# mikostrzewa/AprilSLAM

Hardware: AMD Instinct MI355X
Metric: frames/sec at 1280x720, 20 tags/frame (detection + batched PnP) (higher is better)
Workload: dtype u8/f64

## Files before the change

aprilslam_amd/csrc/aprilslam.hip:

```cpp
#include "../../include/aprilslam.h"

#include <algorithm>
#include <chrono>
#include <cmath>
#include <cstdarg>
#include <cstdio>
#include <cstring>
#include <memory>
#include <string>
#include <type_traits>
#include <vector>

#include "asl_common.h"
#include "tag_standard41h12.inc"
#include "k_wave.inc"

#include "k_threshold.inc"
#include "k_blur.inc"
#include "k_cc.inc"
#include "k_cluster.inc"
#include "k_seg.inc"
#include "k_quad.inc"
#include "k_decode.inc"
#include "k_pnp.inc"
// ... 70 lines not shown
    DevBuf<uint8_t> bgray;
    const uint8_t *qgray = nullptr;
    DevBuf<uint8_t> dbg_thresh;
    DevBuf<unsigned int> dbg_labels;
    DevBuf<unsigned int> parent, sizes;
    DevBuf<unsigned long long> hkeys, points, rootmask, wmask, bmask;
    DevBuf<unsigned int> hcounts, class_lists, stage_pos, frame_cursor, dense_tiles, dense_seg, quad_list;
    DevBuf<unsigned long long> stage_rec;
    DevBuf<uint4> seg_edges;
    unsigned int stage_cap = 0;
    DevBuf<unsigned long long> slot_cluster;
    DevBuf<ClusterRec> clusters;
    DevBuf<QuadRec> quads;
    DevBuf<double> scratch, quadH, wtab, side_mom;
    DevBuf<DetRec> dets;
    DevBuf<unsigned int> frame_ndets, frame_idx, frame_nkeep, frame_off;
    DevBuf<DetOut> out_det;
    DevBuf<PoseOut> out_pose;
    DevBuf<long long> counters;
    DevBuf<float> pnp_corners;
    DevBuf<double> pnp_out;
    DevBuf<uint8_t> pnp_ok;
    DevBuf<uint8_t> gn_ws;
    DevBuf<uint8_t> loc_obs, loc_map;
    DevBuf<uint8_t> solve_out;
    DevBuf<uint8_t> rig_cams;
    DevBuf<uint8_t> cal_ws;
    DevBuf<uint8_t> map_ws, map_lm;
    hipStream_t copy_stream = nullptr, host_stream = nullptr;
    std::vector<hipEvent_t> copy_done;
    hipStream_t aux_stream = nullptr;

    Geom last{};
    unsigned int nslots = 0, max_clusters = 0, max_points = 0, max_dets = 0;
    long long last_counters[CNT__N] = {0};
    bool pending = false;
    const uint8_t *p_frames = nullptr;
    Geom p_geom{};
    hipStream_t p_stream = nullptr;
    bool p_has_cam = false;
    CamDev p_cam{};
    size_t prefetched = 0, nd_guess = 0;
    std::chrono::steady_clock::time_point t_submit, t_enqueued;
    PinnedBuf<long long> pinned_counters;
    PinnedBuf<DetOut> host_det;
    PinnedBuf<PoseOut> host_pose;
    PinnedBuf<unsigned int> host_nkeep;

    int profiling = 0;
    hipEvent_t ev[MAX_STAGES + 1] = {nullptr};
    int nev = 0;
    const char *stage_names[MAX_STAGES] = {nullptr};
    float stage_ms[MAX_STAGES] = {0};
    int nstages = 0;
    float host_ms[4] = {0, 0, 0, 0};

    size_t host_cap() const { return std::min(host_det.n, host_pose.n); }
    ~asl_detector()
    {
        for (hipStream_t s : {aux_stream, copy_stream, host_stream})
            if (s) (void)hipStreamDestroy(s);
        for (hipEvent_t e : copy_done) (void)hipEventDestroy(e);
        for (hipEvent_t e : ev)
            if (e) (void)hipEventDestroy(e);
    }
};

static const char *kVersion = "aprilslam 0.1 gfx950 (HIP, tagStandard41h12)";

extern "C" const char *asl_last_error(void) { return g_err.c_str(); }
extern "C" const char *asl_version(void) { return kVersion; }

// ... 56 lines not shown
    d->fam.nbits = kTag41h12NBits;
    d->fam.width_at_border = kTag41h12WidthAtBorder;
    d->fam.total_width = kTag41h12TotalWidth;
    d->fam.reversed_border = 1;
    d->fam.ncodes = kTag41h12PinnedIds;
    for (int i = 0; i < kTag41h12NBits; i++) { d->fam.bit_x[i] = kTag41h12BitX[i]; d->fam.bit_y[i] = kTag41h12BitY[i]; }
    if (d->codes.ensure(kTag41h12NCodes)) return fail(ASL_ENOMEM, "hipMalloc(code book) failed");
    if (hipMemcpy(d->codes.p, kTag41h12Codes, sizeof(unsigned long long) * kTag41h12NCodes, hipMemcpyHostToDevice) != hipSuccess)
        return fail(ASL_EDEVICE, "hipMemcpy(code book) failed");
    d->fam.codes = d->codes.p;
    if (build_code_index(d.get())) return fail(ASL_ENOMEM, "code-book index allocation failed");
    if (d->wtab.ensure(WEIGHT_TABLE_N)) return fail(ASL_ENOMEM, "hipMalloc(weight table) failed");
    hipLaunchKernelGGL(k_weight_table, dim3((WEIGHT_TABLE_N + 255) / 256), dim3(256), 0, 0, d->wtab.p);
    if (hipDeviceSynchronize() != hipSuccess) return fail(ASL_EDEVICE, "weight table kernel failed");
    (void)hipFuncSetAttribute(reinterpret_cast<const void *>(&k_fit_quads<256, CLASS3_CAP / 256>), hipFuncAttributeMaxDynamicSharedMemorySize, QUAD_LDS_BYTES(CLASS3_CAP));
    *out = d.release();
    return ASL_OK;
}

extern "C" void asl_detector_destroy(asl_detector *d)
{
    if (!d) return;
    (void)hipSetDevice(d->device);
    if (d->pending) (void)hipStreamSynchronize(d->p_stream);
    delete d;
}

extern "C" int asl_detector_set_id_limit(asl_detector *d, int n_ids)
{
    if (!d) return fail(ASL_EINVAL, "detector is NULL");
// ... 53 lines not shown
}

extern "C" int asl_detector_set_pnp_both_minima(asl_detector *d, int enabled)
{
    if (!d) return fail(ASL_EINVAL, "detector is NULL");
    d->pnp_both_minima = enabled ? 1 : 0;
    return ASL_OK;
}

extern "C" int asl_set_profiling(asl_detector *d, int enabled)
{
    if (!d) return fail(ASL_EINVAL, "detector is NULL");
    d->profiling = enabled ? 1 : 0;
    if (enabled)
        for (int i = 0; i <= MAX_STAGES; i++)
            if (!d->ev[i]) HIPCHK(hipEventCreate(&d->ev[i]));
    return ASL_OK;
}

extern "C" int asl_stage_times(asl_detector *d, const char **names, float *ms, int max_n, int *n)
{
    if (!d || !n) return fail(ASL_EINVAL, "NULL argument");
    int k = std::min(max_n, d->nstages);
    for (int i = 0; i < k; i++) { if (names) names[i] = d->stage_names[i]; if (ms) ms[i] = d->stage_ms[i]; }
    static const char *hn[4] = {"host_enqueue", "host_wait", "host_copy", "host_post"};
    for (int i = 0; i < 4 && k < max_n; i++, k++) { if (names) names[k] = hn[i]; if (ms) ms[k] = d->host_ms[i]; }
    *n = k;
    return ASL_OK;
}

static int pnp_tpw(size_t expected)
// ... 61 lines not shown
    bad |= d->quads.ensure(d->max_clusters);
    bad |= d->quad_list.ensure(d->max_clusters);
    bad |= d->quadH.ensure((size_t)10 * d->max_clusters);
    bad |= d->side_mom.ensure((size_t)24 * d->max_clusters);
    bad |= d->points.ensure(d->max_points);
    d->stage_cap = (unsigned int)((double)g.npix * d->points_per_pixel) + 1024u;
    bad |= d->stage_rec.ensure((size_t)B * d->stage_cap);
    bad |= d->stage_pos.ensure((size_t)B * d->stage_cap);
    bad |= d->frame_cursor.ensure(B);
    bad |= d->dense_tiles.ensure(B * count_tiles(g));
    bad |= d->dense_seg.ensure(B * (size_t)seg_nwx(g) * (size_t)((g.sh + SEG_TH - 1) / SEG_TH));
    bad |= d->seg_edges.ensure(B * (size_t)seg_nwx(g) * (size_t)((g.sh + SEG_TH - 1) / SEG_TH));
    bad |= d->scratch.ensure((size_t)d->max_points * 8);
    bad |= d->dets.ensure(d->max_dets);
    bad |= d->frame_ndets.ensure(B);
    bad |= d->frame_nkeep.ensure(B);
    bad |= d->frame_off.ensure(B);
    bad |= d->frame_idx.ensure(B * (size_t)d->dets_per_frame);
    bad |= d->out_det.ensure(d->max_dets);
    bad |= d->out_pose.ensure(d->max_dets);
    bad |= d->counters.ensure(CNT__N);
    if (bad) return fail(ASL_ENOMEM, "device workspace allocation failed (%zu frames of %dx%d)", B, g.sw, g.sh);
    return ASL_OK;
}

#define STAGE(name)                                                        \
    do {                                                                   \
        if (d->profiling && d->nev < MAX_STAGES) {                         \
            d->stage_names[d->nev] = name;                                 \
            HIPCHK(hipEventRecord(d->ev[d->nev], st));                     \
            d->nev++;                                                      \
        }                                                                  \
    } while (0)

static int tag_width(const asl_detector *d, const Geom &g) { return std::max(3, d->fam.width_at_border / g.f); }

// ... 5 lines not shown
                       d->class_lists.p + (size_t)cls * d->max_clusters, d->counters.p, cls, d->max_clusters, CAP, d->points.p, d->qgray, g,
                       tag_width(d, g), want_rev, want_norm, d->scratch.p, d->quads.p, d->wtab.p, d->side_mom.p);
}

static void launch_fit_class(asl_detector *d, const Geom &g, int cls, unsigned int B, hipStream_t st)
{
    const unsigned int qgrid = std::min<unsigned int>(d->max_clusters, std::max<unsigned int>(16384u, 32u * B));
    const unsigned int q2grid = std::min<unsigned int>(d->max_clusters, 2048u);
    switch (cls) {
    case 0: return launch_fit<64, CLASS0_CAP>(d, g, 0, qgrid, st);
    case 1: return launch_fit<128, CLASS1_CAP>(d, g, 1, qgrid, st);
    case 2: return launch_fit<256, CLASS2_CAP>(d, g, 2, q2grid, st);
    case 3: return launch_fit<256, CLASS3_CAP>(d, g, 3, q2grid, st);
    default: return launch_fit<256, 0>(d, g, 4, q2grid, st);
    }
}

static void launch_quad_finish(asl_detector *d, const Geom &g, hipStream_t st)
{
    hipLaunchKernelGGL(k_quad_finish, dim3(std::min<unsigned int>((d->max_clusters + 63) / 64, 4096u)), dim3(256), 0, st, d->quads.p, d->side_mom.p, d->counters.p,
                       d->max_clusters, tag_width(d, g));
}

static int enqueue_detect(asl_detector *d, const uint8_t *d_frames, const Geom &g, hipStream_t st, const CamDev *cam)
{
    dim3 blk(64, 4, 1);
    int thx = (g.sh + TILESZ - 1) / TILESZ;
    unsigned int B = (unsigned int)g.nframes;
    d->nev = 0;
    range_push("S0-S4 gray, decimate, threshold, segmentation, clusters");
// ... 55 lines not shown
    hipLaunchKernelGGL((k_seg_points<SEGP_PCAP_DENSE, SEGP_RUNCAP_DENSE, 1, 2>), dim3(256), dim3(64), 0, st, d->wmask.p, d->bmask.p, g, nwx,
                       d->parent.p, d->sizes.p, d->hkeys.p, d->hcounts.p, d->nslots - 1, d->stage_rec.p, d->stage_pos.p, d->frame_cursor.p,
                       d->stage_cap, d->dense_tiles.p, pty, d->counters.p);
    STAGE("k_cluster_filter");
    hipLaunchKernelGGL(k_cluster_filter, dim3((d->nslots + 1023) / 1024), dim3(1024), 0, st, d->hkeys.p, d->hcounts.p, d->nslots, g,
                       d->clusters.p, d->slot_cluster.p, d->class_lists.p, d->max_clusters, d->max_points, d->counters.p);
    STAGE("k_point_place");
    hipLaunchKernelGGL(k_point_place, dim3(16, B), dim3(256), 0, st, d->stage_rec.p, d->stage_pos.p, d->frame_cursor.p, d->stage_cap,
                       d->slot_cluster.p, d->points.p, d->counters.p);

    range_pop();
    range_push("S5 quad fit");
    for (int cls = 0; cls < NCLASSES; cls++) {
        static const char *const kFitStage[NCLASSES] = {"k_fit_quads<0>", "k_fit_quads<1>", "k_fit_quads<2>", "k_fit_quads<3>", "k_fit_quads<4>"};
        STAGE(kFitStage[cls]);
        launch_fit_class(d, g, cls, B, st);
    }

    STAGE("k_quad_finish");
    launch_quad_finish(d, g, st);
    range_pop();
    range_push("S6-S7 edge refinement, homography, decode");
    STAGE("k_quad_compact");
    hipLaunchKernelGGL(k_quad_compact, dim3((d->max_clusters + 1023) / 1024), dim3(1024), 0, st, d->quads.p, d->counters.p, d->max_clusters,
                       d->quad_list.p);
    unsigned int dgrid = std::min<unsigned int>(d->max_clusters, std::max<unsigned int>(8192u, 64u * B));
    STAGE("k_refine");
    hipLaunchKernelGGL((g.channels == 1 ? k_refine<1> : k_refine<3>), dim3(dgrid), dim3(64), 0, st, d->quads.p, d->counters.p, d->max_clusters, d_frames, g,
                       d->fam.reversed_border ? 1 : 0, d->refine, d->quadH.p, d->quad_list.p, d->side_mom.p);
    STAGE("k_homography");
    hipLaunchKernelGGL(k_homography, dim3(std::min<unsigned int>((d->max_clusters + 31) / 32, 2048u)), dim3(256), 0, st, d->quadH.p, d->counters.p, d->max_clusters,
// ... 4 lines not shown

    range_pop();
    range_push("S9 PnP, S8 de-duplication");
    if (cam) {
        STAGE("k_pnp_dets");
        const int tpw = pnp_tpw(d->nd_guess ? d->nd_guess : (size_t)20 * B);
        hipLaunchKernelGGL(k_pnp_dets, dim3((d->max_dets + tpw - 1) / tpw), dim3(64), 0, st, d->dets.p, d->counters.p, d->max_dets, *cam, tpw);
    }
    STAGE("k_det_dedup");
    {
        const unsigned int cap_f = d->dets_per_frame;
        hipLaunchKernelGGL(k_det_bucket, dim3((d->max_dets + 255) / 256), dim3(256), 0, st, d->dets.p, d->counters.p, d->max_dets, d->frame_ndets.p,
                           d->frame_idx.p, cap_f, d->counters.p);
        hipLaunchKernelGGL(k_det_dedup, dim3(B), dim3(256), 0, st, d->dets.p, d->counters.p, d->frame_ndets.p, d->frame_idx.p, cap_f,
                           d->frame_nkeep.p, d->counters.p);
        hipLaunchKernelGGL(k_det_offsets, dim3(1), dim3(1024), 0, st, d->frame_nkeep.p, B, d->frame_off.p, d->counters.p);
        hipLaunchKernelGGL(k_det_gather, dim3((cap_f + 255) / 256, B), dim3(256), 0, st, d->dets.p, d->frame_idx.p, cap_f, d->frame_nkeep.p,
                           d->frame_off.p, d->out_det.p, d->out_pose.p, d->max_dets, cam ? 1 : 0);
    }
    range_pop();
    if (d->profiling && d->nev <= MAX_STAGES) HIPCHK(hipEventRecord(d->ev[d->nev], st));
    HIPCHK(hipGetLastError());
    return ASL_OK;
}

static CamDev make_cam(const asl_detector *d, const double *K, const double *dist, int n_dist, double tag_size)
{
    CamDev c;
    c.both_minima = d->pnp_both_minima; c.pad = 0;
    c.fx = K[0]; c.fy = K[4]; c.cx = K[2]; c.cy = K[5];
    c.k1 = c.k2 = c.p1 = c.p2 = c.k3 = 0;
    if (dist && n_dist >= 4) { c.k1 = dist[0]; c.k2 = dist[1]; c.p1 = dist[2]; c.p2 = dist[3]; }
    if (dist && n_dist >= 5) c.k3 = dist[4];
    c.half = (double)(float)(tag_size / 2);
    return c;
}

using clk = std::chrono::steady_clock;
static float msf(clk::time_point a, clk::time_point b) { return std::chrono::duration<float, std::milli>(b - a).count(); }

static int ensure_host_out(asl_detector *d, size_t want, size_t nframes)
{
    HIPCHK(d->host_nkeep.ensure(nframes, hipHostMallocDefault));
    if (want <= d->host_cap()) return ASL_OK;
    d->host_det.release(); d->host_pose.release();
    want = std::max<size_t>(want * 2, 4096);
    HIPCHK(d->host_det.ensure(want, hipHostMallocNonCoherent));
    HIPCHK(d->host_pose.ensure(want, hipHostMallocNonCoherent));
    return ASL_OK;
}

static int submit_batch(asl_detector *d, const uint8_t *d_frames, const Geom &g, hipStream_t st, const CamDev *cam)
{
    if (d->pending) return fail(ASL_EINVAL, "a batch is already in flight on this detector: collect it first");
    int rc = ensure_workspace(d, g);
    if (rc) return rc;
    d->t_submit = clk::now();
    rc = enqueue_detect(d, d_frames, g, st, cam);
    if (rc) return rc;
    HIPCHK(d->pinned_counters.ensure(CNT__N, hipHostMallocDefault));
    HIPCHK(hipMemcpyAsync(d->pinned_counters.p, d->counters.p, sizeof(long long) * CNT__N, hipMemcpyDeviceToHost, st));
    d->prefetched = 0;
    rc = ensure_host_out(d, std::min<size_t>(d->nd_guess, d->max_dets), (size_t)g.nframes);
    if (rc) return rc;
    HIPCHK(hipMemcpyAsync(d->host_nkeep.p, d->frame_nkeep.p, sizeof(unsigned int) * (size_t)g.nframes, hipMemcpyDeviceToHost, st));
    if (d->nd_guess > 0) {
        size_t guess = std::min<size_t>(d->nd_guess, d->max_dets);
        HIPCHK(hipMemcpyAsync(d->host_det.p, d->out_det.p, guess * sizeof(DetOut), hipMemcpyDeviceToHost, st));
        if (cam) HIPCHK(hipMemcpyAsync(d->host_pose.p, d->out_pose.p, guess * sizeof(PoseOut), hipMemcpyDeviceToHost, st));
        d->prefetched = guess;
    }
    d->pending = true;
    d->p_frames = d_frames; d->p_geom = g; d->p_stream = st; d->p_has_cam = cam != nullptr;
    if (cam) d->p_cam = *cam;
    d->t_enqueued = clk::now();
    return ASL_OK;
}

static int collect_batch(asl_detector *d, asl_detection *out, asl_pose *poses, int max_out, int *n_per_frame, int *n_out)
{
    if (!d->pending) return fail(ASL_EINVAL, "no batch in flight on this detector");
    const Geom g = d->p_geom;
    hipStream_t st = d->p_stream;
    const CamDev *cam = d->p_has_cam ? &d->p_cam : nullptr;
    clk::time_point t0 = d->t_submit, t1 = d->t_enqueued, t2 = t1;
    for (int attempt = 0; attempt < 4; attempt++) {
        if (attempt > 0) {
            d->pending = false;
            d->nd_guess = 0;
            int rc = submit_batch(d, d->p_frames, g, st, cam);
            if (rc) return rc;
        }
        HIPCHK(hipStreamSynchronize(st));
        t2 = clk::now();
        memcpy(d->last_counters, d->pinned_counters.p, sizeof(long long) * CNT__N);
        d->last = g;
        long long *c = d->last_counters;
        if (c[CNT_UF_GUARD]) {
            d->pending = false;
            return fail(ASL_ECAPACITY, "a union-find loop hit its iteration guard (%lld times): labels of this batch are not trustworthy", c[CNT_UF_GUARD]);
        }
        bool again = false;
        if (c[CNT_OVERFLOW_HASH]) { d->hash_slots_per_frame *= 4; again = true; }
        if (c[CNT_OVERFLOW_CLUSTERS] || c[CNT_NCLUSTERS] > (long long)d->max_clusters) { d->clusters_per_frame *= 4; again = true; }
        if (c[CNT_OVERFLOW_POINTS]) { d->points_per_pixel *= 2; again = true; }
        if (c[CNT_OVERFLOW_DETS]) { d->dets_per_frame *= 4; again = true; }
        if (again) {
            if (attempt == 3) {
                d->pending = false;
                return fail(ASL_ECAPACITY, "work buffers still overflow after growing (hash %lld clusters %lld points %lld dets %lld)",
// ... 1 lines not shown
            }
            continue;
        }
        break;
    }
    d->pending = false;
    if (d->profiling) {
        d->nstages = d->nev;
        for (int i = 0; i < d->nev; i++) HIPCHK(hipEventElapsedTime(&d->stage_ms[i], d->ev[i], d->ev[i + 1]));
    }
    if (d->last_counters[CNT_DEDUP_LIMIT])
        return fail(ASL_ECAPACITY, "%lld frame(s) hold more than %d detections: the de-duplication does not sort that many", d->last_counters[CNT_DEDUP_LIMIT], DEDUP_MAX);
    size_t nd = (size_t)d->last_counters[CNT_NKEEP];
    if (nd > d->max_dets) nd = d->max_dets;
    if (nd > d->prefetched) {
        size_t have = d->prefetched;
        if (nd > d->host_cap()) have = 0;
        int rc = ensure_host_out(d, nd, (size_t)g.nframes);
        if (rc) return rc;
        HIPCHK(hipMemcpy(d->host_det.p + have, d->out_det.p + have, (nd - have) * sizeof(DetOut), hipMemcpyDeviceToHost));
        if (cam) HIPCHK(hipMemcpy(d->host_pose.p + have, d->out_pose.p + have, (nd - have) * sizeof(PoseOut), hipMemcpyDeviceToHost));
    }
    d->nd_guess = nd + nd / 4 + 256;
    clk::time_point t3 = clk::now();
    static_assert(sizeof(DetOut) == sizeof(asl_detection) && sizeof(PoseOut) == sizeof(asl_pose), "device results are copied verbatim");
    int total = (int)nd;
    int nw = std::min(total, max_out);
    if (out && nw > 0) memcpy(out, d->host_det.p, (size_t)nw * sizeof(asl_detection));
    if (poses && cam && nw > 0) memcpy(poses, d->host_pose.p, (size_t)nw * sizeof(asl_pose));
    if (n_per_frame) for (int f = 0; f < g.nframes; f++) n_per_frame[f] = (int)d->host_nkeep.p[f];
    if (n_out) *n_out = total;
    d->host_ms[0] = msf(t0, t1); d->host_ms[1] = msf(t1, t2); d->host_ms[2] = msf(t2, t3); d->host_ms[3] = msf(t3, clk::now());
    return ASL_OK;
}

static int check_n_dist(int n_dist)
{
    if (n_dist != 0 && n_dist != 4 && n_dist != 5) return fail(ASL_EINVAL, "n_dist must be 0, 4 or 5");
    return ASL_OK;
}

static int check_device_args(asl_detector *d, const void *d_frames, int n_frames, int channels, int w, int h, int stride, size_t frame_pitch,
                             int n_dist, Geom *g)
{
    if (!d || !d_frames) return fail(ASL_EINVAL, "NULL detector or frames");
// ... 19 lines not shown
extern "C" int asl_collect_batch(asl_detector *d, asl_detection *out, asl_pose *poses, int max_out, int *n_per_frame, int *n_out)
{
    if (!d) return fail(ASL_EINVAL, "NULL detector");
    if (max_out < 0 || (max_out > 0 && !out)) return fail(ASL_EINVAL, "out is NULL");
    HIPCHK(hipSetDevice(d->device));
    return collect_batch(d, out, poses, max_out, n_per_frame, n_out);
}

extern "C" int asl_collect_batch_view(asl_detector *d, const asl_detection **out, const asl_pose **poses, const uint32_t **n_per_frame, int *n_out)
{
    if (!d || !out || !n_per_frame || !n_out) return fail(ASL_EINVAL, "NULL argument");
    HIPCHK(hipSetDevice(d->device));
    const bool with_poses = d->p_has_cam;
    int rc = collect_batch(d, nullptr, nullptr, 0, nullptr, n_out);
    if (rc) return rc;
    *out = reinterpret_cast<const asl_detection *>(d->host_det.p);
    if (poses) *poses = with_poses ? reinterpret_cast<const asl_pose *>(d->host_pose.p) : nullptr;
    *n_per_frame = d->host_nkeep.p;
    return ASL_OK;
}

extern "C" int asl_detect_batch_device(asl_detector *d, const void *d_frames, int n_frames, int channels, int w, int h, int stride,
                                       size_t frame_pitch, void *stream, const double *K, const double *dist, int n_dist,
                                       double tag_size, asl_detection *out, asl_pose *poses, int max_out, int *n_per_frame, int *n_out)
{
    if (max_out < 0 || (max_out > 0 && !out)) return fail(ASL_EINVAL, "out is NULL");
    int rc = asl_submit_batch_device(d, d_frames, n_frames, channels, w, h, stride, frame_pitch, stream, K, dist, n_dist, tag_size);
    if (rc) return rc;
    return collect_batch(d, out, poses, max_out, n_per_frame, n_out);
}

#define HOST_CHUNK_FRAMES 64
static hipError_t copy_frames(asl_detector *d, const uint8_t *const *frames, int f0, int f1, size_t pitch, hipStream_t st)
// ... 714 lines not shown
```

aprilslam_amd/csrc/k_dedup.inc:

```

#define DEDUP_MAX 1024

struct DetOut {
    int32_t id, hamming;
    float margin;
    int32_t frame;
    double center[2];
    double corners[4][2];
};
struct PoseOut {
    double rvec[3], tvec[3], T[16];
    int32_t ok, reserved;
};

__device__ __forceinline__ bool dd_seg_intersect(const double *a, const double *b, const double *c, const double *d)
{
    double d1 = (b[0] - a[0]) * (c[1] - a[1]) - (b[1] - a[1]) * (c[0] - a[0]);
    double d2 = (b[0] - a[0]) * (d[1] - a[1]) - (b[1] - a[1]) * (d[0] - a[0]);
    double d3 = (d[0] - c[0]) * (a[1] - c[1]) - (d[1] - c[1]) * (a[0] - c[0]);
    double d4 = (d[0] - c[0]) * (b[1] - c[1]) - (d[1] - c[1]) * (b[0] - c[0]);
    return ((d1 > 0) != (d2 > 0)) && ((d3 > 0) != (d4 > 0));
}
__device__ __forceinline__ bool dd_point_in_quad(const double q[4][2], const double *p)
{
    int pos = 0, neg = 0;
    for (int i = 0; i < 4; i++) {
        const double *a = q[i], *b = q[(i + 1) & 3];
        double c = (b[0] - a[0]) * (p[1] - a[1]) - (b[1] - a[1]) * (p[0] - a[0]);
// ... 125 lines not shown
        const bool f = i < n && s_alive[i];
        const unsigned long long mask = __ballot(f);
        const unsigned int prefix = (unsigned int)__popcll(mask & ((1ull << lane) - 1ull));
        if (lane == 0) s_wave[wid] = (unsigned int)__popcll(mask);
        __syncthreads();
        unsigned int off = s_base;
        for (int w = 0; w < wid; w++) off += s_wave[w];
        if (f) fidx[off + prefix] = s_idx[i];
        __syncthreads();
        if (tid == 0) s_base += s_wave[0] + s_wave[1] + s_wave[2] + s_wave[3];
        __syncthreads();
    }
    if (tid == 0) frame_nkeep[fr] = s_base;
}

__global__ void __launch_bounds__(1024) k_det_offsets(const unsigned int *__restrict__ frame_nkeep, unsigned int nframes, unsigned int *__restrict__ frame_off,
                                                      long long *wcounters)
{
    __shared__ unsigned int s_w[16], s_carry;
    const int tid = threadIdx.x, lane = tid & 63, wid = tid >> 6;
    if (tid == 0) s_carry = 0;
    __syncthreads();
    for (unsigned int start = 0; start < nframes; start += 1024) {
        const unsigned int i = start + tid;
        const unsigned int v = i < nframes ? frame_nkeep[i] : 0u;
        unsigned int incl = v;
#pragma unroll
        for (int off = 1; off < 64; off <<= 1) {
            unsigned int o = __shfl_up(incl, off);
            if (lane >= off) incl += o;
        }
        if (lane == 63) s_w[wid] = incl;
        __syncthreads();
        unsigned int base = s_carry;
        for (int w = 0; w < wid; w++) base += s_w[w];
        if (i < nframes) frame_off[i] = base + incl - v;
        __syncthreads();
        if (tid == 1023) s_carry = base + incl;
        __syncthreads();
    }
    if (tid == 0) wcounters[CNT_NKEEP] = (long long)s_carry;
}

__global__ void __launch_bounds__(256) k_det_gather(const DetRec *__restrict__ dets, const unsigned int *__restrict__ frame_idx, unsigned int cap_f,
                                                    const unsigned int *__restrict__ frame_nkeep, const unsigned int *__restrict__ frame_off,
                                                    DetOut *__restrict__ out_det, PoseOut *__restrict__ out_pose, unsigned int max_out, int with_pose)
{
    const unsigned int fr = blockIdx.y;
    const unsigned int j = blockIdx.x * blockDim.x + threadIdx.x;
    if (j >= frame_nkeep[fr]) return;
    const unsigned int at = frame_off[fr] + j;
    if (at >= max_out) return;
    const DetRec &r = dets[frame_idx[(size_t)fr * cap_f + j]];
    DetOut o;
    o.id = r.id; o.hamming = r.hamming; o.margin = r.margin; o.frame = r.frame;
    o.center[0] = r.center[0]; o.center[1] = r.center[1];
    for (int i = 0; i < 4; i++) { o.corners[i][0] = r.corners[i][0]; o.corners[i][1] = r.corners[i][1]; }
    out_det[at] = o;
    if (with_pose) {
        PoseOut p;
        for (int i = 0; i < 3; i++) { p.rvec[i] = r.rvec[i]; p.tvec[i] = r.tvec[i]; }
        for (int i = 0; i < 16; i++) p.T[i] = r.T[i];
        p.ok = r.pose_ok; p.reserved = 0;
        out_pose[at] = p;
    }
}
```

aprilslam_amd/csrc/k_quad.inc:

```

__device__ const unsigned int kCombo4of10[210] = {
    0x003210u, 0x014210u, 0x074310u, 0x1c4320u, 0x544321u, 0x025210u, 0x085310u, 0x1d5320u, 0x555321u, 0x0d5410u,
    0x225420u, 0x5a5421u, 0x315430u, 0x695431u, 0x8c5432u, 0x036210u, 0x096310u, 0x1e6320u, 0x566321u, 0x0e6410u,
    0x236420u, 0x5b6421u, 0x326430u, 0x6a6431u, 0x8d6432u, 0x126510u, 0x276520u, 0x5f6521u, 0x366530u, 0x6e6531u,
    0x916532u, 0x406540u, 0x786541u, 0x9b6542u, 0xaf6543u, 0x047210u, 0x0a7310u, 0x1f7320u, 0x577321u, 0x0f7410u,
    0x247420u, 0x5c7421u, 0x337430u, 0x6b7431u, 0x8e7432u, 0x137510u, 0x287520u, 0x607521u, 0x377530u, 0x6f7531u,
    0x927532u, 0x417540u, 0x797541u, 0x9c7542u, 0xb07543u, 0x167610u, 0x2b7620u, 0x637621u, 0x3a7630u, 0x727631u,
    0x957632u, 0x447640u, 0x7c7641u, 0x9f7642u, 0xb37643u, 0x4a7650u, 0x827651u, 0xa57652u, 0xb97653u, 0xc37654u,
    0x058210u, 0x0b8310u, 0x208320u, 0x588321u, 0x108410u, 0x258420u, 0x5d8421u, 0x348430u, 0x6c8431u, 0x8f8432u,
    0x148510u, 0x298520u, 0x618521u, 0x388530u, 0x708531u, 0x938532u, 0x428540u, 0x7a8541u, 0x9d8542u, 0xb18543u,
    0x178610u, 0x2c8620u, 0x648621u, 0x3b8630u, 0x738631u, 0x968632u, 0x458640u, 0x7d8641u, 0xa08642u, 0xb48643u,
    0x4b8650u, 0x838651u, 0xa68652u, 0xba8653u, 0xc48654u, 0x198710u, 0x2e8720u, 0x668721u, 0x3d8730u, 0x758731u,
    0x988732u, 0x478740u, 0x7f8741u, 0xa28742u, 0xb68743u, 0x4d8750u, 0x858751u, 0xa88752u, 0xbc8753u, 0xc68754u,
    0x508760u, 0x888761u, 0xab8762u, 0xbf8763u, 0xc98764u, 0xcd8765u, 0x069210u, 0x0c9310u, 0x219320u, 0x599321u,
    0x119410u, 0x269420u, 0x5e9421u, 0x359430u, 0x6d9431u, 0x909432u, 0x159510u, 0x2a9520u, 0x629521u, 0x399530u,
    0x719531u, 0x949532u, 0x439540u, 0x7b9541u, 0x9e9542u, 0xb29543u, 0x189610u, 0x2d9620u, 0x659621u, 0x3c9630u,
    0x749631u, 0x979632u, 0x469640u, 0x7e9641u, 0xa19642u, 0xb59643u, 0x4c9650u, 0x849651u, 0xa79652u, 0xbb9653u,
    0xc59654u, 0x1a9710u, 0x2f9720u, 0x679721u, 0x3e9730u, 0x769731u, 0x999732u, 0x489740u, 0x809741u, 0xa39742u,
    0xb79743u, 0x4e9750u, 0x869751u, 0xa99752u, 0xbd9753u, 0xc79754u, 0x519760u, 0x899761u, 0xac9762u, 0xc09763u,
    0xca9764u, 0xce9765u, 0x1b9810u, 0x309820u, 0x689821u, 0x3f9830u, 0x779831u, 0x9a9832u, 0x499840u, 0x819841u,
    0xa49842u, 0xb89843u, 0x4f9850u, 0x879851u, 0xaa9852u, 0xbe9853u, 0xc89854u, 0x529860u, 0x8a9861u, 0xad9862u,
    0xc19863u, 0xcb9864u, 0xcf9865u, 0x539870u, 0x8b9871u, 0xae9872u, 0xc29873u, 0xcc9874u, 0xd09875u, 0xd19876u,
};
__device__ const unsigned short kPairOff[12] = {0, 0, 0, 0, 0, 7, 20, 41, 72, 115, 172, 245};
// ... 247 lines not shown
struct FitShared {
    int *wave, *base;
    int *tmpi; long long *tmpl; double *tmpd;
    int *maxidx;
    double *pnx, *pny;
    int *found, *best; double *thresh;
};

template <int NT, int PPT>
struct FitFetch {
    static constexpr int NREC = PPT > 0 ? PPT : 1;
    const unsigned int *class_list;
    const ClusterRec *clusters;
    const unsigned long long *points;
    unsigned int last;
    unsigned int ci_nx, ci_nn, ci_n3;
    ClusterRec cl_nx, cl_nn;
    unsigned long long recs_nx[NREC];

    __device__ __forceinline__ void load_recs()
    {
        const int tid = threadIdx.x;
#pragma unroll
        for (int e = 0; e < NREC; e++) {
            int i = tid + e * NT;
            recs_nx[e] = i < (int)cl_nx.count ? points[(size_t)cl_nx.offset + i] : 0ull;
        }
    }
    __device__ __forceinline__ void open(const unsigned int *class_list_, const ClusterRec *clusters_, const unsigned long long *points_, unsigned int ncl)
    {
        class_list = class_list_; clusters = clusters_; points = points_; last = ncl - 1;
        if constexpr (PPT > 0) {
            const unsigned int G = gridDim.x;
            ci_nx = class_list[blockIdx.x];
            ci_nn = class_list[min(blockIdx.x + G, last)];
            ci_n3 = class_list[min(blockIdx.x + 2 * G, last)];
            cl_nx = clusters[ci_nx];
            cl_nn = clusters[ci_nn];
            load_recs();
        }
    }
    __device__ __forceinline__ void advance(unsigned int li, unsigned int &ci, ClusterRec &cl, unsigned long long (&recs)[NREC])
    {
        if constexpr (PPT > 0) {
            ci = ci_nx; cl = cl_nx;
#pragma unroll
            for (int e = 0; e < NREC; e++) recs[e] = recs_nx[e];
            ci_nx = ci_nn; cl_nx = cl_nn;
            load_recs();
            ci_nn = ci_n3;
            cl_nn = clusters[ci_nn];
            ci_n3 = class_list[min(li + 3 * gridDim.x, last)];
        } else {
            ci = class_list[li];
            cl = clusters[ci];
        }
    }
};


template <int NT, int PPT>
__device__ __forceinline__ int fit_box_polarity(const FitShared &sh, const unsigned long long (&recs)[PPT > 0 ? PPT : 1], const unsigned long long *seg, int n,
                                                 int tag_width, int want_reversed, int want_normal, float &cx, float &cy)
{
    const int tid = threadIdx.x;
    int xmin = 0x7FFFFFFF, xmax = 0, ymin = 0x7FFFFFFF, ymax = 0, sgx = 0, sgy = 0;
    long long sxg = 0;
// ... 269 lines not shown
        if (len < 0) len += sz;
        if (len > 8) {
            int t = len / 6;
            i0 = (i0 + t) % sz;
            i1 = (i1 + sz - t) % sz;
        }
        double M[6];
        fit_moments_dev(mom, i0, i1, M);
        double *out = side_mom + ((size_t)ci * 4 + tid) * 6;
#pragma unroll
        for (int k = 0; k < 6; k++) out[k] = M[k];
    }
}

template <int NT, int PPT>
__global__ void __launch_bounds__(NT) k_fit_quads(const ClusterRec *__restrict__ clusters, const unsigned int *__restrict__ class_list,
                                                  const long long *__restrict__ counters, int cls, unsigned int max_clusters, int cap,
                                                  unsigned long long *points, const uint8_t *__restrict__ dgray, Geom g, int tag_width,
                                                  int want_reversed, int want_normal, double *scratch, QuadRec *quads, const double *__restrict__ wtab,
                                                  double *__restrict__ side_mom)
{
    extern __shared__ __align__(16) unsigned char smem[];
    __shared__ int s_wave[4], s_base, s_n;
    __shared__ int s_maxidx[MAX_NMAXIMA], s_best[4];
    __shared__ double s_thresh;
    __shared__ double s_tmpd[4];
    __shared__ long long s_tmpl[4];
    __shared__ int s_tmpi[4];
    __shared__ double s_pnx[NPAIR], s_pny[NPAIR];
    const FitShared sh = {s_wave, &s_base, s_tmpi, s_tmpl, s_tmpd, s_maxidx, s_pnx, s_pny, &s_n, s_best, &s_thresh};
    const int tid = threadIdx.x;
    PHASE_DECL();
    if (batch_poisoned(counters)) return;
    long long ncl64 = counters[CNT_CLASS(cls)];
    unsigned int ncl = ncl64 > (long long)max_clusters ? max_clusters : (unsigned int)ncl64;
    if (blockIdx.x >= ncl) return;
    FitFetch<NT, PPT> fetch;
    fetch.open(class_list, clusters, points, ncl);

    for (unsigned int li = blockIdx.x; li < ncl; li += gridDim.x) {
        __syncthreads();
        PHASE_INIT();
        unsigned int ci;
        ClusterRec cl;
        unsigned long long recs[FitFetch<NT, PPT>::NREC];
        fetch.advance(li, ci, cl, recs);
        if (tid == 0) { quads[ci].valid = 0; quads[ci].key = cl.key; quads[ci].reversed_border = 0; }
        const int n = (int)cl.count;
        if (n < 24) continue;
        unsigned long long *seg = points + cl.offset;
        FitStore st;
        if constexpr (PPT > 0) st = fit_store_lds(smem, cap);
        else st = fit_store_slab(seg, scratch + (size_t)cl.offset * 8, n);

        float cx, cy;
// ... 14 lines not shown
        fit_window_errors<NT>(st, mom, ksz);
        PHASE(5);
        const int nmax = fit_maxima<NT>(st, sh, sz);
        if (nmax < 4) continue;
        PHASE(6);
        const bool won = fit_corner_search<NT>(st, sh, mom, nmax);
        PHASE(7);
        if (!won) continue;
        fit_side_moments(sh, mom, side_mom, ci);
        if (tid == 0) quads[ci].valid = 2;
        PHASE(8);
    }
    PHASE_FLUSH(0);
}

__global__ void __launch_bounds__(256) k_quad_finish(QuadRec *__restrict__ quads, const double *__restrict__ side_mom, const long long *__restrict__ counters,
                                                     unsigned int max_clusters, int tag_width)
{
    if (batch_poisoned(counters)) return;
    const long long ncl64 = counters[CNT_NCLUSTERS];
    const unsigned int ncl = ncl64 > (long long)max_clusters ? max_clusters : (unsigned int)ncl64;
    const int lane = threadIdx.x & 63, l = lane & 3;
    for (unsigned int c0 = blockIdx.x * 64u; c0 < ncl; c0 += gridDim.x * 64u) {
        const unsigned int ci = c0 + (threadIdx.x >> 2);
        const bool pending = ci < ncl && quads[ci].valid == 2;
        if (!__any(pending)) continue;
        double M[6];
        const double *in = side_mom + ((size_t)(pending ? ci : 0) * 4 + l) * 6;
#pragma unroll
        for (int k = 0; k < 6; k++) M[k] = pending ? in[k] : 1.0;
// ... 66 lines not shown
```

Baseline: 393,900.

## Pack results into one transfer block and fuse fit and offset kernels

Counters, per-frame keep counts, detections and poses now sit in one contiguous device result block, so submission needs a single async D2H copy instead of up to four. The prefix-offset kernel is folded into the gather kernel: each block recomputes its frame's base by summing earlier frames. The class-3 and class-4 quad-fit launches are merged into one kernel that splits its grid in half. This cuts launch and copy-enqueue overhead at the cost of redundant prefix sums per block, a more complex front/back result layout, and a fixed even grid split between the two classes.

Result: no change. 397,300, median of 6 (+0.9%).

```diff
diff --git a/aprilslam_amd/csrc/aprilslam.hip b/aprilslam_amd/csrc/aprilslam.hip
--- a/aprilslam_amd/csrc/aprilslam.hip
+++ b/aprilslam_amd/csrc/aprilslam.hip
@@ -108,10 +108,11 @@
     DevBuf<QuadRec> quads;
     DevBuf<double> scratch, quadH, wtab, side_mom;
     DevBuf<DetRec> dets;
-    DevBuf<unsigned int> frame_ndets, frame_idx, frame_nkeep, frame_off;
-    DevBuf<DetOut> out_det;
-    DevBuf<PoseOut> out_pose;
-    DevBuf<long long> counters;
+    DevBuf<unsigned int> frame_ndets, frame_idx;
+    DevBuf<uint8_t> result;
+    ResView<long long> counters;
+    ResView<unsigned int> frame_nkeep;
+    size_t res_hdr = 0;
     DevBuf<float> pnp_corners;
     DevBuf<double> pnp_out;
     DevBuf<uint8_t> pnp_ok;
@@ -136,10 +137,11 @@
     CamDev p_cam{};
     size_t prefetched = 0, nd_guess = 0;
     std::chrono::steady_clock::time_point t_submit, t_enqueued;
-    PinnedBuf<long long> pinned_counters;
-    PinnedBuf<DetOut> host_det;
-    PinnedBuf<PoseOut> host_pose;
-    PinnedBuf<unsigned int> host_nkeep;
+    PinnedBuf<uint8_t> host_res;
+    const long long *host_counters = nullptr;
+    DetOut *host_det = nullptr;
+    PoseOut *host_pose = nullptr;
+    unsigned int *host_nkeep = nullptr;
 
     int profiling = 0;
     hipEvent_t ev[MAX_STAGES + 1] = {nullptr};
@@ -149,7 +151,7 @@
     int nstages = 0;
     float host_ms[4] = {0, 0, 0, 0};
 
-    size_t host_cap() const { return std::min(host_det.n, host_pose.n); }
+    size_t host_cap() const { return host_res.n > res_hdr ? (host_res.n - res_hdr) / RES_REC_BYTES : 0; }
     ~asl_detector()
     {
         for (hipStream_t s : {aux_stream, copy_stream, host_stream})
@@ -236,6 +238,7 @@
     hipLaunchKernelGGL(k_weight_table, dim3((WEIGHT_TABLE_N + 255) / 256), dim3(256), 0, 0, d->wtab.p);
     if (hipDeviceSynchronize() != hipSuccess) return fail(ASL_EDEVICE, "weight table kernel failed");
     (void)hipFuncSetAttribute(reinterpret_cast<const void *>(&k_fit_quads<256, CLASS3_CAP / 256>), hipFuncAttributeMaxDynamicSharedMemorySize, QUAD_LDS_BYTES(CLASS3_CAP));
+    (void)hipFuncSetAttribute(reinterpret_cast<const void *>(&k_fit_quads_large), hipFuncAttributeMaxDynamicSharedMemorySize, QUAD_LDS_BYTES(CLASS3_CAP));
     *out = d.release();
     return ASL_OK;
 }
@@ -319,7 +322,7 @@
     d->profiling = enabled ? 1 : 0;
     if (enabled)
         for (int i = 0; i <= MAX_STAGES; i++)
-            if (!d->ev[i]) HIPCHK(hipEventCreate(&d->ev[i]));
+            if (!d->ev[i]) HIPCHK(hipEventCreateWithFlags(&d->ev[i], hipEventDisableSystemFence));
     return ASL_OK;
 }
 
@@ -411,12 +414,11 @@
     bad |= d->scratch.ensure((size_t)d->max_points * 8);
     bad |= d->dets.ensure(d->max_dets);
     bad |= d->frame_ndets.ensure(B);
-    bad |= d->frame_nkeep.ensure(B);
-    bad |= d->frame_off.ensure(B);
     bad |= d->frame_idx.ensure(B * (size_t)d->dets_per_frame);
-    bad |= d->out_det.ensure(d->max_dets);
-    bad |= d->out_pose.ensure(d->max_dets);
-    bad |= d->counters.ensure(CNT__N);
+    d->res_hdr = res_hdr_bytes(B);
+    bad |= d->result.ensure(d->res_hdr + (size_t)d->max_dets * RES_REC_BYTES);
+    d->counters.p = (long long *)d->result.p;
+    d->frame_nkeep.p = (unsigned int *)(d->result.p + sizeof(long long) * CNT__N);
     if (bad) return fail(ASL_ENOMEM, "device workspace allocation failed (%zu frames of %dx%d)", B, g.sw, g.sh);
     return ASL_OK;
 }
@@ -452,6 +454,15 @@
     case 3: return launch_fit<256, CLASS3_CAP>(d, g, 3, q2grid, st);
     default: return launch_fit<256, 0>(d, g, 4, q2grid, st);
     }
+}
+
+static void launch_fit_large(asl_detector *d, const Geom &g, hipStream_t st)
+{
+    const unsigned int q2grid = std::min<unsigned int>(d->max_clusters, 2048u);
+    hipLaunchKernelGGL(k_fit_quads_large, dim3(2 * q2grid), dim3(256), QUAD_LDS_BYTES(CLASS3_CAP), st, d->clusters.p,
+                       d->class_lists.p + (size_t)3 * d->max_clusters, d->class_lists.p + (size_t)4 * d->max_clusters, d->counters.p, d->max_clusters,
+                       d->points.p, d->qgray, g, tag_width(d, g), d->fam.reversed_border ? 1 : 0, d->fam.reversed_border ? 0 : 1, d->scratch.p, d->quads.p,
+                       d->wtab.p, d->side_mom.p);
 }
 
 static void launch_quad_finish(asl_detector *d, const Geom &g, hipStream_t st)
@@ -537,7 +548,8 @@
     for (int cls = 0; cls < NCLASSES; cls++) {
         static const char *const kFitStage[NCLASSES] = {"k_fit_quads<0>", "k_fit_quads<1>", "k_fit_quads<2>", "k_fit_quads<3>", "k_fit_quads<4>"};
         STAGE(kFitStage[cls]);
-        launch_fit_class(d, g, cls, B, st);
+        if (cls < 3) launch_fit_class(d, g, cls, B, st);
+        else if (cls == 3) launch_fit_large(d, g, st);
     }
 
     STAGE("k_quad_finish");
@@ -572,9 +584,8 @@
                            d->frame_idx.p, cap_f, d->counters.p);
         hipLaunchKernelGGL(k_det_dedup, dim3(B), dim3(256), 0, st, d->dets.p, d->counters.p, d->frame_ndets.p, d->frame_idx.p, cap_f,
                            d->frame_nkeep.p, d->counters.p);
-        hipLaunchKernelGGL(k_det_offsets, dim3(1), dim3(1024), 0, st, d->frame_nkeep.p, B, d->frame_off.p, d->counters.p);
         hipLaunchKernelGGL(k_det_gather, dim3((cap_f + 255) / 256, B), dim3(256), 0, st, d->dets.p, d->frame_idx.p, cap_f, d->frame_nkeep.p,
-                           d->frame_off.p, d->out_det.p, d->out_pose.p, d->max_dets, cam ? 1 : 0);
+                           B, d->counters.p, ResLayout{d->result.p + d->res_hdr, (unsigned int)d->prefetched, d->max_dets}, cam ? 1 : 0);
     }
     range_pop();
     if (d->profiling && d->nev <= MAX_STAGES) HIPCHK(hipEventRecord(d->ev[d->nev], st));
@@ -597,15 +608,21 @@
 using clk = std::chrono::steady_clock;
 static float msf(clk::time_point a, clk::time_point b) { return std::chrono::duration<float, std::milli>(b - a).count(); }
 
-static int ensure_host_out(asl_detector *d, size_t want, size_t nframes)
-{
-    HIPCHK(d->host_nkeep.ensure(nframes, hipHostMallocDefault));
-    if (want <= d->host_cap()) return ASL_OK;
-    d->host_det.release(); d->host_pose.release();
+static int ensure_host_out(asl_detector *d, size_t want)
+{
+    if (d->host_res.p && want <= d->host_cap()) return ASL_OK;
+    d->host_res.release();
     want = std::max<size_t>(want * 2, 4096);
-    HIPCHK(d->host_det.ensure(want, hipHostMallocNonCoherent));
-    HIPCHK(d->host_pose.ensure(want, hipHostMallocNonCoherent));
-    return ASL_OK;
+    HIPCHK(d->host_res.ensure(d->res_hdr + want * RES_REC_BYTES, hipHostMallocNonCoherent));
+    return ASL_OK;
+}
+
+static void set_host_layout(asl_detector *d, size_t front)
+{
+    d->host_counters = (const long long *)d->host_res.p;
+    d->host_nkeep = (unsigned int *)(d->host_res.p + sizeof(long long) * CNT__N);
+    d->host_det = (DetOut *)(d->host_res.p + d->res_hdr);
+    d->host_pose = (PoseOut *)(d->host_res.p + d->res_hdr + front * sizeof(DetOut));
 }
 
 static int submit_batch(asl_detector *d, const uint8_t *d_frames, const Geom &g, hipStream_t st, const CamDev *cam)
@@ -614,20 +631,14 @@
     int rc = ensure_workspace(d, g);
     if (rc) return rc;
     d->t_submit = clk::now();
+    d->prefetched = std::min<size_t>(d->nd_guess, d->max_dets);
+    rc = ensure_host_out(d, d->prefetched);
+    if (rc) return rc;
+    set_host_layout(d, d->prefetched);
     rc = enqueue_detect(d, d_frames, g, st, cam);
     if (rc) return rc;
-    HIPCHK(d->pinned_counters.ensure(CNT__N, hipHostMallocDefault));
-    HIPCHK(hipMemcpyAsync(d->pinned_counters.p, d->counters.p, sizeof(long long) * CNT__N, hipMemcpyDeviceToHost, st));
-    d->prefetched = 0;
-    rc = ensure_host_out(d, std::min<size_t>(d->nd_guess, d->max_dets), (size_t)g.nframes);
-    if (rc) return rc;
-    HIPCHK(hipMemcpyAsync(d->host_nkeep.p, d->frame_nkeep.p, sizeof(unsigned int) * (size_t)g.nframes, hipMemcpyDeviceToHost, st));
-    if (d->nd_guess > 0) {
-        size_t guess = std::min<size_t>(d->nd_guess, d->max_dets);
-        HIPCHK(hipMemcpyAsync(d->host_det.p, d->out_det.p, guess * sizeof(DetOut), hipMemcpyDeviceToHost, st));
-        if (cam) HIPCHK(hipMemcpyAsync(d->host_pose.p, d->out_pose.p, guess * sizeof(PoseOut), hipMemcpyDeviceToHost, st));
-        d->prefetched = guess;
-    }
+    HIPCHK(hipMemcpyAsync(d->host_res.p, d->result.p, d->res_hdr + d->prefetched * (sizeof(DetOut) + (cam ? sizeof(PoseOut) : 0)),
+                          hipMemcpyDeviceToHost, st));
     d->pending = true;
     d->p_frames = d_frames; d->p_geom = g; d->p_stream = st; d->p_has_cam = cam != nullptr;
     if (cam) d->p_cam = *cam;
@@ -651,7 +662,7 @@
         }
         HIPCHK(hipStreamSynchronize(st));
         t2 = clk::now();
-        memcpy(d->last_counters, d->pinned_counters.p, sizeof(long long) * CNT__N);
+        memcpy(d->last_counters, d->host_counters, sizeof(long long) * CNT__N);
         d->last = g;
         long long *c = d->last_counters;
         if (c[CNT_UF_GUARD]) {
@@ -683,21 +694,30 @@
     size_t nd = (size_t)d->last_counters[CNT_NKEEP];
     if (nd > d->max_dets) nd = d->max_dets;
     if (nd > d->prefetched) {
-        size_t have = d->prefetched;
-        if (nd > d->host_cap()) have = 0;
-        int rc = ensure_host_out(d, nd, (size_t)g.nframes);
+        const ResLayout dev{d->result.p + d->res_hdr, (unsigned int)d->prefetched, d->max_dets};
+        const size_t front = d->prefetched;
+        const bool grow = nd > d->host_cap();
+        int rc = ensure_host_out(d, nd);
         if (rc) return rc;
-        HIPCHK(hipMemcpy(d->host_det.p + have, d->out_det.p + have, (nd - have) * sizeof(DetOut), hipMemcpyDeviceToHost));
-        if (cam) HIPCHK(hipMemcpy(d->host_pose.p + have, d->out_pose.p + have, (nd - have) * sizeof(PoseOut), hipMemcpyDeviceToHost));
+        set_host_layout(d, nd);
+        if (grow) {
+            HIPCHK(hipMemcpy(d->host_res.p, d->result.p, d->res_hdr, hipMemcpyDeviceToHost));
+            if (front) HIPCHK(hipMemcpy(d->host_det, dev.det(0), front * sizeof(DetOut), hipMemcpyDeviceToHost));
+        }
+        HIPCHK(hipMemcpy(d->host_det + front, dev.det(front), (nd - front) * sizeof(DetOut), hipMemcpyDeviceToHost));
+        if (cam) {
+            if (front) HIPCHK(hipMemcpy(d->host_pose, dev.pose(0), front * sizeof(PoseOut), hipMemcpyDeviceToHost));
+            HIPCHK(hipMemcpy(d->host_pose + front, dev.pose(front), (nd - front) * sizeof(PoseOut), hipMemcpyDeviceToHost));
+        }
     }
     d->nd_guess = nd + nd / 4 + 256;
     clk::time_point t3 = clk::now();
     static_assert(sizeof(DetOut) == sizeof(asl_detection) && sizeof(PoseOut) == sizeof(asl_pose), "device results are copied verbatim");
     int total = (int)nd;
     int nw = std::min(total, max_out);
-    if (out && nw > 0) memcpy(out, d->host_det.p, (size_t)nw * sizeof(asl_detection));
-    if (poses && cam && nw > 0) memcpy(poses, d->host_pose.p, (size_t)nw * sizeof(asl_pose));
-    if (n_per_frame) for (int f = 0; f < g.nframes; f++) n_per_frame[f] = (int)d->host_nkeep.p[f];
+    if (out && nw > 0) memcpy(out, d->host_det, (size_t)nw * sizeof(asl_detection));
+    if (poses && cam && nw > 0) memcpy(poses, d->host_pose, (size_t)nw * sizeof(asl_pose));
+    if (n_per_frame) for (int f = 0; f < g.nframes; f++) n_per_frame[f] = (int)d->host_nkeep[f];
     if (n_out) *n_out = total;
     d->host_ms[0] = msf(t0, t1); d->host_ms[1] = msf(t1, t2); d->host_ms[2] = msf(t2, t3); d->host_ms[3] = msf(t3, clk::now());
     return ASL_OK;
@@ -747,9 +767,9 @@
     const bool with_poses = d->p_has_cam;
     int rc = collect_batch(d, nullptr, nullptr, 0, nullptr, n_out);
     if (rc) return rc;
-    *out = reinterpret_cast<const asl_detection *>(d->host_det.p);
-    if (poses) *poses = with_poses ? reinterpret_cast<const asl_pose *>(d->host_pose.p) : nullptr;
-    *n_per_frame = d->host_nkeep.p;
+    *out = reinterpret_cast<const asl_detection *>(d->host_det);
+    if (poses) *poses = with_poses ? reinterpret_cast<const asl_pose *>(d->host_pose) : nullptr;
+    *n_per_frame = d->host_nkeep;
     return ASL_OK;
 }
 
diff --git a/aprilslam_amd/csrc/k_dedup.inc b/aprilslam_amd/csrc/k_dedup.inc
--- a/aprilslam_amd/csrc/k_dedup.inc
+++ b/aprilslam_amd/csrc/k_dedup.inc
@@ -12,6 +12,27 @@
     double rvec[3], tvec[3], T[16];
     int32_t ok, reserved;
 };
+
+#define RES_REC_BYTES (sizeof(DetOut) + sizeof(PoseOut))
+static inline size_t res_hdr_bytes(size_t nframes) { return (sizeof(long long) * CNT__N + sizeof(unsigned int) * nframes + 255) & ~(size_t)255; }
+template <typename T>
+struct ResView {
+    T *p = nullptr;
+};
+struct ResLayout {
+    uint8_t *body;
+    unsigned int front, max_out;
+    __host__ __device__ DetOut *det(size_t at) const
+    {
+        return at < front ? (DetOut *)body + at : (DetOut *)(body + front * RES_REC_BYTES) + (at - front);
+    }
+    __host__ __device__ PoseOut *pose(size_t at) const
+    {
+        return at < front ? (PoseOut *)(body + front * sizeof(DetOut)) + at
+                          : (PoseOut *)(body + front * RES_REC_BYTES + (size_t)(max_out - front) * sizeof(DetOut)) + (at - front);
+    }
+};
+static_assert(sizeof(DetOut) % 8 == 0 && sizeof(PoseOut) % 8 == 0, "every piece of the result block stays 8-byte aligned");
 
 __device__ __forceinline__ bool dd_seg_intersect(const double *a, const double *b, const double *c, const double *d)
 {
@@ -167,54 +188,43 @@
     if (tid == 0) frame_nkeep[fr] = s_base;
 }
 
-__global__ void __launch_bounds__(1024) k_det_offsets(const unsigned int *__restrict__ frame_nkeep, unsigned int nframes, unsigned int *__restrict__ frame_off,
-                                                      long long *wcounters)
-{
-    __shared__ unsigned int s_w[16], s_carry;
-    const int tid = threadIdx.x, lane = tid & 63, wid = tid >> 6;
-    if (tid == 0) s_carry = 0;
-    __syncthreads();
-    for (unsigned int start = 0; start < nframes; start += 1024) {
-        const unsigned int i = start + tid;
-        const unsigned int v = i < nframes ? frame_nkeep[i] : 0u;
-        unsigned int incl = v;
-#pragma unroll
-        for (int off = 1; off < 64; off <<= 1) {
-            unsigned int o = __shfl_up(incl, off);
-            if (lane >= off) incl += o;
-        }
-        if (lane == 63) s_w[wid] = incl;
-        __syncthreads();
-        unsigned int base = s_carry;
-        for (int w = 0; w < wid; w++) base += s_w[w];
-        if (i < nframes) frame_off[i] = base + incl - v;
-        __syncthreads();
-        if (tid == 1023) s_carry = base + incl;
-        __syncthreads();
-    }
-    if (tid == 0) wcounters[CNT_NKEEP] = (long long)s_carry;
+__device__ __forceinline__ unsigned int dd_count_before(const unsigned int *__restrict__ frame_nkeep, unsigned int n)
+{
+    __shared__ unsigned int s_part[4];
+    unsigned int v = 0;
+    for (unsigned int i = threadIdx.x; i < n; i += 256) v += frame_nkeep[i];
+    v = wave_scan<true>(v, 0u, [](unsigned int a, unsigned int b) { return a + b; });
+    if ((threadIdx.x & 63) == 0) s_part[threadIdx.x >> 6] = v;
+    __syncthreads();
+    return s_part[0] + s_part[1] + s_part[2] + s_part[3];
 }
 
 __global__ void __launch_bounds__(256) k_det_gather(const DetRec *__restrict__ dets, const unsigned int *__restrict__ frame_idx, unsigned int cap_f,
-                                                    const unsigned int *__restrict__ frame_nkeep, const unsigned int *__restrict__ frame_off,
-                                                    DetOut *__restrict__ out_det, PoseOut *__restrict__ out_pose, unsigned int max_out, int with_pose)
+                                                    const unsigned int *__restrict__ frame_nkeep, unsigned int nframes, long long *wcounters,
+                                                    ResLayout out, int with_pose)
 {
     const unsigned int fr = blockIdx.y;
     const unsigned int j = blockIdx.x * blockDim.x + threadIdx.x;
+    const bool first = fr == 0 && blockIdx.x == 0;
+    unsigned int before = dd_count_before(frame_nkeep, first ? nframes : fr);
+    if (first) {
+        if (threadIdx.x == 0) wcounters[CNT_NKEEP] = (long long)before;
+        before = 0;
+    }
     if (j >= frame_nkeep[fr]) return;
-    const unsigned int at = frame_off[fr] + j;
-    if (at >= max_out) return;
+    const unsigned int at = before + j;
+    if (at >= out.max_out) return;
     const DetRec &r = dets[frame_idx[(size_t)fr * cap_f + j]];
     DetOut o;
     o.id = r.id; o.hamming = r.hamming; o.margin = r.margin; o.frame = r.frame;
     o.center[0] = r.center[0]; o.center[1] = r.center[1];
     for (int i = 0; i < 4; i++) { o.corners[i][0] = r.corners[i][0]; o.corners[i][1] = r.corners[i][1]; }
-    out_det[at] = o;
+    *out.det(at) = o;
     if (with_pose) {
         PoseOut p;
         for (int i = 0; i < 3; i++) { p.rvec[i] = r.rvec[i]; p.tvec[i] = r.tvec[i]; }
         for (int i = 0; i < 16; i++) p.T[i] = r.T[i];
         p.ok = r.pose_ok; p.reserved = 0;
-        out_pose[at] = p;
-    }
-}
+        *out.pose(at) = p;
+    }
+}
diff --git a/aprilslam_amd/csrc/k_quad.inc b/aprilslam_amd/csrc/k_quad.inc
--- a/aprilslam_amd/csrc/k_quad.inc
+++ b/aprilslam_amd/csrc/k_quad.inc
@@ -285,6 +285,7 @@
     const ClusterRec *clusters;
     const unsigned long long *points;
     unsigned int last;
+    unsigned int G;
     unsigned int ci_nx, ci_nn, ci_n3;
     ClusterRec cl_nx, cl_nn;
     unsigned long long recs_nx[NREC];
@@ -298,14 +299,14 @@
             recs_nx[e] = i < (int)cl_nx.count ? points[(size_t)cl_nx.offset + i] : 0ull;
         }
     }
-    __device__ __forceinline__ void open(const unsigned int *class_list_, const ClusterRec *clusters_, const unsigned long long *points_, unsigned int ncl)
+    __device__ __forceinline__ void open(const unsigned int *class_list_, const ClusterRec *clusters_, const unsigned long long *points_, unsigned int ncl,
+                                         unsigned int wg, unsigned int nwg)
     {
-        class_list = class_list_; clusters = clusters_; points = points_; last = ncl - 1;
+        class_list = class_list_; clusters = clusters_; points = points_; last = ncl - 1; G = nwg;
         if constexpr (PPT > 0) {
-            const unsigned int G = gridDim.x;
-            ci_nx = class_list[blockIdx.x];
-            ci_nn = class_list[min(blockIdx.x + G, last)];
-            ci_n3 = class_list[min(blockIdx.x + 2 * G, last)];
+            ci_nx = class_list[wg];
+            ci_nn = class_list[min(wg + G, last)];
+            ci_n3 = class_list[min(wg + 2 * G, last)];
             cl_nx = clusters[ci_nx];
             cl_nn = clusters[ci_nn];
             load_recs();
@@ -321,7 +322,7 @@
             load_recs();
             ci_nn = ci_n3;
             cl_nn = clusters[ci_nn];
-            ci_n3 = class_list[min(li + 3 * gridDim.x, last)];
+            ci_n3 = class_list[min(li + 3 * G, last)];
         } else {
             ci = class_list[li];
             cl = clusters[ci];
@@ -621,11 +622,11 @@
 }
 
 template <int NT, int PPT>
-__global__ void __launch_bounds__(NT) k_fit_quads(const ClusterRec *__restrict__ clusters, const unsigned int *__restrict__ class_list,
-                                                  const long long *__restrict__ counters, int cls, unsigned int max_clusters, int cap,
-                                                  unsigned long long *points, const uint8_t *__restrict__ dgray, Geom g, int tag_width,
-                                                  int want_reversed, int want_normal, double *scratch, QuadRec *quads, const double *__restrict__ wtab,
-                                                  double *__restrict__ side_mom)
+__device__ __forceinline__ void fit_quads_list(const ClusterRec *__restrict__ clusters, const unsigned int *__restrict__ class_list,
+                                               const long long *__restrict__ counters, int cls, unsigned int max_clusters, int cap,
+                                               unsigned long long *points, const uint8_t *__restrict__ dgray, const Geom &g, int tag_width,
+                                               int want_reversed, int want_normal, double *scratch, QuadRec *quads, const double *__restrict__ wtab,
+                                               double *__restrict__ side_mom, unsigned int wg, unsigned int nwg)
 {
     extern __shared__ __align__(16) unsigned char smem[];
     __shared__ int s_wave[4], s_base, s_n;
@@ -641,11 +642,11 @@
     if (batch_poisoned(counters)) return;
     long long ncl64 = counters[CNT_CLASS(cls)];
     unsigned int ncl = ncl64 > (long long)max_clusters ? max_clusters : (unsigned int)ncl64;
-    if (blockIdx.x >= ncl) return;
+    if (wg >= ncl) return;
     FitFetch<NT, PPT> fetch;
-    fetch.open(class_list, clusters, points, ncl);
-
-    for (unsigned int li = blockIdx.x; li < ncl; li += gridDim.x) {
+    fetch.open(class_list, clusters, points, ncl, wg, nwg);
+
+    for (unsigned int li = wg; li < ncl; li += nwg) {
         __syncthreads();
         PHASE_INIT();
         unsigned int ci;
@@ -690,6 +691,32 @@
     PHASE_FLUSH(0);
 }
 
+template <int NT, int PPT>
+__global__ void __launch_bounds__(NT) k_fit_quads(const ClusterRec *__restrict__ clusters, const unsigned int *__restrict__ class_list,
+                                                  const long long *__restrict__ counters, int cls, unsigned int max_clusters, int cap,
+                                                  unsigned long long *points, const uint8_t *__restrict__ dgray, Geom g, int tag_width,
+                                                  int want_reversed, int want_normal, double *scratch, QuadRec *quads, const double *__restrict__ wtab,
+                                                  double *__restrict__ side_mom)
+{
+    fit_quads_list<NT, PPT>(clusters, class_list, counters, cls, max_clusters, cap, points, dgray, g, tag_width, want_reversed, want_normal, scratch, quads,
+                            wtab, side_mom, blockIdx.x, gridDim.x);
+}
+
+__global__ void __launch_bounds__(256) k_fit_quads_large(const ClusterRec *__restrict__ clusters, const unsigned int *__restrict__ list3,
+                                                         const unsigned int *__restrict__ list4, const long long *__restrict__ counters,
+                                                         unsigned int max_clusters, unsigned long long *points, const uint8_t *__restrict__ dgray, Geom g,
+                                                         int tag_width, int want_reversed, int want_normal, double *scratch, QuadRec *quads,
+                                                         const double *__restrict__ wtab, double *__restrict__ side_mom)
+{
+    const unsigned int half = gridDim.x / 2;
+    if (blockIdx.x < half)
+        fit_quads_list<256, CLASS3_CAP / 256>(clusters, list3, counters, 3, max_clusters, CLASS3_CAP, points, dgray, g, tag_width, want_reversed, want_normal,
+                                              scratch, quads, wtab, side_mom, blockIdx.x, half);
+    else
+        fit_quads_list<256, 0>(clusters, list4, counters, 4, max_clusters, 0, points, dgray, g, tag_width, want_reversed, want_normal, scratch, quads, wtab,
+                               side_mom, blockIdx.x - half, half);
+}
+
 __global__ void __launch_bounds__(256) k_quad_finish(QuadRec *__restrict__ quads, const double *__restrict__ side_mom, const long long *__restrict__ counters,
                                                      unsigned int max_clusters, int tag_width)
 {
```
